# asmirnou/watsor

Measured on NVIDIA H100. Metric: aggregate detection FPS on synthetic 640x480 streams, higher is better.
Workload: dtype f32

## Files before the change

### watsor_b200/csrc/kernels_tc.cu

```cuda
#include <cuda.h>

#include <algorithm>
#include <cstdlib>
#include <cstring>

#include "kernels_tc.cuh"
#include "tc_common.cuh"

namespace {

struct TcArgs {
  const float* scale;
  const float* offset;
  void* out;
  float* enc;
  float* logits;
  int M, N, n_pad, K;
  int block_n, stages, k_blocks;
  int splits, kb_per;
  float* partial;
  int* tile_counters;
  const void* residual;
  int conv, cpb, conv_kw, conv_pad_t, conv_pad_l;
  int ring_bytes;
  int rows_per_tile;
  int act, is_head, anchors_per_loc, row_off, n_box, num_anchors, ncp1, hw;
};

__device__ __forceinline__ void tma_load_4d_tc(uint32_t dst, const CUtensorMap* map, uint32_t bar, int c0, int c1, int c2,
                                               int c3) {
  asm volatile(
      "cp.async.bulk.tensor.4d.shared::cluster.global.mbarrier::complete_tx::bytes [%0], [%1, {%3, %4, %5, %6}], [%2];" ::
          "r"(dst),
      "l"(map), "r"(bar), "r"(c0), "r"(c1), "r"(c2), "r"(c3)
      : "memory");
}

__device__ __forceinline__ void cluster_sync_all() {
  asm volatile("barrier.cluster.arrive.release.aligned;\nbarrier.cluster.wait.acquire.aligned;" ::: "memory");
}
__device__ __forceinline__ uint32_t cluster_ctarank() {
  uint32_t r;
  asm volatile("mov.u32 %0, %%cluster_ctarank;" : "=r"(r));
  return r;
}
__device__ __forceinline__ float4 ld_dsmem128(uint32_t addr, uint32_t rank) {
  uint32_t ra;
  asm volatile("mapa.shared::cluster.u32 %0, %1, %2;" : "=r"(ra) : "r"(addr), "r"(rank));
  float4 v;
  asm volatile("ld.shared::cluster.v4.f32 {%0,%1,%2,%3}, [%4];" : "=f"(v.x), "=f"(v.y), "=f"(v.z), "=f"(v.w) : "r"(ra));
  return v;
}

template <bool TF32>
__device__ __forceinline__ void copy_out_row(const TcArgs& g, const uint8_t* smem, int pitch, int r, int m0, int n0,
                                             int lane, int members, int reduce) {
  const int mm = m0 + r;
  const uint32_t src = smem_u32(smem) + (uint32_t)(r * pitch * 4);
  size_t hr = 0;
  if (g.is_head) {
    const int f = mm / g.hw;
    hr = (size_t)f * g.num_anchors + g.row_off + (size_t)(mm - f * g.hw) * g.anchors_per_loc;
  }
  for (int j = lane * 4; j < g.block_n; j += 128) {
    const int nn = n0 + j;
    if (nn >= g.N) break;
    float4 y;
    if (reduce) {
      float4 p[8];
      if (members == 1) {
        p[0] = lds128(src + (uint32_t)(j * 4));
      } else {
#pragma unroll
        for (int z = 0; z < 8; ++z)
          if (z < members) p[z] = ld_dsmem128(src + (uint32_t)(j * 4), (uint32_t)z);
      }
      y = p[0];
#pragma unroll
      for (int z = 1; z < 8; ++z)
        if (z < members) y = make_float4(__fadd_rn(y.x, p[z].x), __fadd_rn(y.y, p[z].y), __fadd_rn(y.z, p[z].z), __fadd_rn(y.w, p[z].w));
      const float4 sc = *reinterpret_cast<const float4*>(g.scale + nn), of = *reinterpret_cast<const float4*>(g.offset + nn);
      y = make_float4(affine_rn(y.x, sc.x, of.x), affine_rn(y.y, sc.y, of.y), affine_rn(y.z, sc.z, of.z), affine_rn(y.w, sc.w, of.w));
      if (g.act == WB_ACT_RELU6) y = make_float4(relu6f(y.x), relu6f(y.y), relu6f(y.z), relu6f(y.w));
    } else {
      y = lds128(src + (uint32_t)(j * 4));
    }
    if (g.is_head) {
      const float ys[4] = {y.x, y.y, y.z, y.w};
#pragma unroll
      for (int e = 0; e < 4; ++e) {
        const int c = nn + e;
        if (c >= g.N) break;
        if (c < g.n_box)
          g.enc[hr * 4 + c] = ys[e];
        else
          g.logits[hr * g.ncp1 + (c - g.n_box)] = ys[e];
      }
    } else if (TF32) {
      if (g.residual != nullptr) {
        const float4 rr = *reinterpret_cast<const float4*>(reinterpret_cast<const float*>(g.residual) + (size_t)mm * g.N + nn);
        y = make_float4(__fadd_rn(y.x, rr.x), __fadd_rn(y.y, rr.y), __fadd_rn(y.z, rr.z), __fadd_rn(y.w, rr.w));
      }
      *reinterpret_cast<float4*>(reinterpret_cast<float*>(g.out) + (size_t)mm * g.N + nn) = y;
    } else {
      ActIO<__nv_bfloat16>::st4(reinterpret_cast<__nv_bfloat16*>(g.out) + (size_t)mm * g.N + nn, y);
    }
  }
}

constexpr int GEMM_THREADS = 288;
constexpr int GEMM_PRODUCER_WARP = 8;

__device__ __forceinline__ void wg_bar_sync(int wg) { asm volatile("bar.sync %0, 128;" ::"r"(2 + wg) : "memory"); }

template <int MODE, int BN>
__global__ void __launch_bounds__(GEMM_THREADS, 1)
    k_gemm_tc(const __grid_constant__ CUtensorMap map_a, const __grid_constant__ CUtensorMap map_b,
              const __grid_constant__ CUtensorMap map_b_lo, TcArgs g) {
  constexpr bool TF32 = MODE != 0;
  constexpr bool X3 = MODE == 2;
  constexpr int ELEM = TF32 ? 4 : 2;
  constexpr int K_PER_BLOCK = ROW_BYTES / ELEM;
  constexpr int B_TILE_BYTES = BN * ROW_BYTES;
  constexpr int SLOTS = X3 ? 2 : 1;
  constexpr int STAGE_BYTES = (A_TILE_BYTES + B_TILE_BYTES) * SLOTS;
  extern __shared__ __align__(1024) uint8_t smem_raw[];
  uint8_t* smem = reinterpret_cast<uint8_t*>((reinterpret_cast<uintptr_t>(smem_raw) + 1023) & ~(uintptr_t)1023);
  uint64_t* full = reinterpret_cast<uint64_t*>(smem + (size_t)g.ring_bytes);
  uint64_t* empty = full + g.stages;

  const int warp = threadIdx.x >> 5, lane = threadIdx.x & 31;
  const int m0 = blockIdx.x * g.rows_per_tile, n0 = blockIdx.y * BN;
  const int kb0 = blockIdx.z * g.kb_per;
  const int nkb = min(g.k_blocks, kb0 + g.kb_per) - kb0;

  if (threadIdx.x == 0) {
    for (int s = 0; s < g.stages; ++s) {
      mbar_init(smem_u32(&full[s]), 1);
      mbar_init(smem_u32(&empty[s]), 2);
    }
    fence_barrier_init();
  }
  __syncthreads();

  float acc[BN / 2];
#pragma unroll
  for (int i = 0; i < BN / 2; ++i) acc[i] = 0.f;

  if (warp == GEMM_PRODUCER_WARP) {
    if (elect_one()) {
      asm volatile("prefetch.tensormap [%0];" ::"l"(&map_a) : "memory");
      asm volatile("prefetch.tensormap [%0];" ::"l"(&map_b) : "memory");
      for (int it = 0; it < nkb; ++it) {
        const int kb = kb0 + it;
        const int s = it % g.stages;
        const uint32_t ph = (it / g.stages) & 1;
        mbar_wait(smem_u32(&empty[s]), ph ^ 1);
        uint8_t* st = smem + (size_t)s * STAGE_BYTES;
        const uint32_t bar = smem_u32(&full[s]);
        if (g.conv) {
          mbar_expect_tx(bar, g.rows_per_tile * ROW_BYTES + B_TILE_BYTES * SLOTS);
          const int tap = kb / g.cpb, cb = kb - tap * g.cpb;
          const int ky = tap / g.conv_kw, kx = tap - ky * g.conv_kw;
          tma_load_4d_tc(smem_u32(st), &map_a, bar, cb * K_PER_BLOCK, kx - g.conv_pad_l, ky - g.conv_pad_t, m0 / g.hw);
        } else {
          mbar_expect_tx(bar, A_TILE_BYTES + B_TILE_BYTES * SLOTS);
          tma_load_2d(smem_u32(st), &map_a, bar, kb * K_PER_BLOCK, m0);
        }
        uint8_t* sb = st + A_TILE_BYTES * SLOTS;
        tma_load_2d(smem_u32(sb), &map_b, bar, kb * K_PER_BLOCK, n0);
        if (X3) tma_load_2d(smem_u32(sb + B_TILE_BYTES), &map_b_lo, bar, kb * K_PER_BLOCK, n0);
      }
    }
  } else {
    const int wg = warp >> 2, t = threadIdx.x & 127;
    float part[X3 ? BN / 2 : 1];
    for (int it = 0; it < nkb; ++it) {
      const int s = it % g.stages;
      mbar_wait(smem_u32(&full[s]), (it / g.stages) & 1);
      const uint32_t st = smem_u32(smem + (size_t)s * STAGE_BYTES);
      const uint32_t a_hi = st + (uint32_t)(wg * 64 * ROW_BYTES), a_lo = a_hi + A_TILE_BYTES;
      const uint32_t b_hi = st + (uint32_t)(A_TILE_BYTES * SLOTS), b_lo = b_hi + B_TILE_BYTES;
      if (X3) {
#pragma unroll
        for (int i = t; i < 64 * ROW_BYTES / 16; i += 128) split_tf32(a_hi + (uint32_t)(i * 16), a_lo + (uint32_t)(i * 16));
        fence_proxy_async();
        wg_bar_sync(wg);
        wg_x3_kblock_sum<BN>(acc, part, a_hi, a_lo, b_hi, b_lo);
      } else {
        wgmma_fence();
        wg_mma_kblock<TF32, false, BN>(acc, a_hi, a_lo, b_hi, b_lo, 1u);
        wgmma_commit();
        wgmma_wait_all();
      }
      wg_bar_sync(wg);
      if (t == 0) mbar_arrive(smem_u32(&empty[s]));
    }
  }

  const int pitch = BN + 4;
  __syncthreads();
  if (warp < GEMM_PRODUCER_WARP) {
    const int row = (warp >> 2) * 64 + (warp & 3) * 16 + (lane >> 2);
    const uint32_t stg = smem_u32(smem) + (uint32_t)((row * pitch + 2 * (lane & 3)) * 4);
#pragma unroll
    for (int i = 0; i < BN / 2; i += 4) {
      const uint32_t c = (uint32_t)((i >> 2) * 8 * 4);
      asm volatile("st.shared.v2.f32 [%0], {%1, %2};" ::"r"(stg + c), "f"(acc[i]), "f"(acc[i + 1]) : "memory");
      asm volatile("st.shared.v2.f32 [%0], {%1, %2};" ::"r"(stg + c + (uint32_t)(8 * pitch * 4)), "f"(acc[i + 2]), "f"(acc[i + 3])
                   : "memory");
    }
  }
  __syncthreads();
  const int n_warps = blockDim.x >> 5;
  const int rows = min(g.rows_per_tile, g.M - m0);
  if (g.splits > 1) {
    cluster_sync_all();
    const int z = (int)cluster_ctarank();
    for (int r = z + g.splits * warp; r < rows; r += n_warps * g.splits)
      copy_out_row<TF32>(g, smem, pitch, r, m0, n0, lane, g.splits, 1);
    __syncwarp();
    cluster_sync_all();
  } else if (g.is_head) {
    for (int r = warp; r < rows; r += n_warps) copy_out_row<TF32>(g, smem, pitch, r, m0, n0, lane, 1, 1);
  } else {
    const int c4n = g.block_n >> 2;
    const int items = rows * c4n;
    const int T = (int)blockDim.x;
    const uint32_t sbase = smem_u32(smem);
    int inc_r = T / c4n, inc_c = T - inc_r * c4n;
    int r_it = (int)threadIdx.x / c4n, c_it = (int)threadIdx.x - r_it * c4n;
    if (TF32 && inc_r >= 1) {
      inc_c = 0;
      if ((int)threadIdx.x >= inc_r * c4n) r_it = rows;
    }
    if (inc_c == 0 && TF32) {
      const int nn = n0 + c_it * 4;
      if (nn < g.N && r_it < rows) {
        const float4 sc = __ldg(reinterpret_cast<const float4*>(g.scale + nn)), of = __ldg(reinterpret_cast<const float4*>(g.offset + nn));
        const bool relu = g.act == WB_ACT_RELU6;
        uint32_t sp = sbase + (uint32_t)((r_it * pitch + c_it * 4) * 4);
        const uint32_t sstep = (uint32_t)(inc_r * pitch * 4);
        float* op = reinterpret_cast<float*>(g.out) + (size_t)(m0 + r_it) * g.N + nn;
        const float* rp = g.residual != nullptr ? reinterpret_cast<const float*>(g.residual) + (size_t)(m0 + r_it) * g.N + nn : nullptr;
        const size_t gstep = (size_t)inc_r * g.N;
        int r = r_it;
        for (; r + 3 * inc_r < rows; r += 4 * inc_r) {
          float4 y[4], rs[4];
#pragma unroll
          for (int u = 0; u < 4; ++u) {
            y[u] = lds128(sp + u * sstep);
            if (rp != nullptr) rs[u] = *reinterpret_cast<const float4*>(rp + u * gstep);
          }
#pragma unroll
          for (int u = 0; u < 4; ++u) {
            float4 v = make_float4(affine_rn(y[u].x, sc.x, of.x), affine_rn(y[u].y, sc.y, of.y), affine_rn(y[u].z, sc.z, of.z),
                                   affine_rn(y[u].w, sc.w, of.w));
            if (relu) v = make_float4(relu6f(v.x), relu6f(v.y), relu6f(v.z), relu6f(v.w));
            if (rp != nullptr) v = make_float4(__fadd_rn(v.x, rs[u].x), __fadd_rn(v.y, rs[u].y), __fadd_rn(v.z, rs[u].z), __fadd_rn(v.w, rs[u].w));
            *reinterpret_cast<float4*>(op + u * gstep) = v;
          }
          sp += 4 * sstep;
          op += 4 * gstep;
          if (rp != nullptr) rp += 4 * gstep;
        }
        for (; r < rows; r += inc_r) {
          const float4 y = lds128(sp);
          float4 v = make_float4(affine_rn(y.x, sc.x, of.x), affine_rn(y.y, sc.y, of.y), affine_rn(y.z, sc.z, of.z), affine_rn(y.w, sc.w, of.w));
          if (relu) v = make_float4(relu6f(v.x), relu6f(v.y), relu6f(v.z), relu6f(v.w));
          if (rp != nullptr) {
            const float4 r4 = *reinterpret_cast<const float4*>(rp);
            v = make_float4(__fadd_rn(v.x, r4.x), __fadd_rn(v.y, r4.y), __fadd_rn(v.z, r4.z), __fadd_rn(v.w, r4.w));
            rp += gstep;
          }
          *reinterpret_cast<float4*>(op) = v;
          sp += sstep;
          op += gstep;
        }
      }
    } else
    for (int i0 = threadIdx.x; i0 < items; i0 += 4 * T) {
      float4 y[4], sc[4], of[4];
      int rr[4], cc[4];
#pragma unroll
      for (int u = 0; u < 4; ++u) {
        rr[u] = r_it;
        cc[u] = c_it * 4;
        if (i0 + T * u < items && n0 + cc[u] < g.N) {
          y[u] = lds128(sbase + (uint32_t)((rr[u] * pitch + cc[u]) * 4));
          sc[u] = __ldg(reinterpret_cast<const float4*>(g.scale + n0 + cc[u]));
          of[u] = __ldg(reinterpret_cast<const float4*>(g.offset + n0 + cc[u]));
        }
        r_it += inc_r;
        c_it += inc_c;
        if (c_it >= c4n) {
          c_it -= c4n;
          ++r_it;
        }
      }
#pragma unroll
      for (int u = 0; u < 4; ++u) {
        const int nn = n0 + cc[u];
        if (i0 + T * u >= items || nn >= g.N) continue;
        const size_t o = (size_t)(m0 + rr[u]) * g.N + nn;
        y[u] = make_float4(affine_rn(y[u].x, sc[u].x, of[u].x), affine_rn(y[u].y, sc[u].y, of[u].y),
                           affine_rn(y[u].z, sc[u].z, of[u].z), affine_rn(y[u].w, sc[u].w, of[u].w));
        if (g.act == WB_ACT_RELU6) y[u] = make_float4(relu6f(y[u].x), relu6f(y[u].y), relu6f(y[u].z), relu6f(y[u].w));
        if (TF32) {
          if (g.residual != nullptr) {
            const float4 r4 = *reinterpret_cast<const float4*>(reinterpret_cast<const float*>(g.residual) + o);
            y[u] = make_float4(__fadd_rn(y[u].x, r4.x), __fadd_rn(y[u].y, r4.y), __fadd_rn(y[u].z, r4.z), __fadd_rn(y[u].w, r4.w));
          }
          *reinterpret_cast<float4*>(reinterpret_cast<float*>(g.out) + o) = y[u];
        } else {
          ActIO<__nv_bfloat16>::st4(reinterpret_cast<__nv_bfloat16*>(g.out) + o, y[u]);
        }
      }
    }
  }
}


typedef CUresult (*EncodeTiledFn)(CUtensorMap*, CUtensorMapDataType, cuuint32_t, void*, const cuuint64_t*,
                                  const cuuint64_t*, const cuuint32_t*, const cuuint32_t*, CUtensorMapInterleave,
                                  CUtensorMapSwizzle, CUtensorMapL2promotion, CUtensorMapFloatOOBfill);

EncodeTiledFn encode_fn() {
  static EncodeTiledFn fn = nullptr;
  if (!fn) {
    void* p = nullptr;
    cudaDriverEntryPointQueryResult q;
    if (cudaGetDriverEntryPoint("cuTensorMapEncodeTiled", &p, cudaEnableDefault, &q) == cudaSuccess &&
        q == cudaDriverEntryPointSuccess)
      fn = reinterpret_cast<EncodeTiledFn>(p);
  }
  return fn;
}

bool make_map(CUtensorMap* map, const void* base, int elem_bytes, int rows, int k, int box_rows, std::string* err) {
  EncodeTiledFn fn = encode_fn();
  if (!fn) {
    *err = "cuTensorMapEncodeTiled is not available from the driver";
    return false;
  }
  cuuint64_t dims[2] = {(cuuint64_t)k, (cuuint64_t)rows};
  cuuint64_t strides[1] = {(cuuint64_t)k * elem_bytes};
  cuuint32_t box[2] = {(cuuint32_t)(ROW_BYTES / elem_bytes), (cuuint32_t)box_rows};
  cuuint32_t estr[2] = {1, 1};
  CUresult r = fn(map, elem_bytes == 2 ? CU_TENSOR_MAP_DATA_TYPE_BFLOAT16 : CU_TENSOR_MAP_DATA_TYPE_FLOAT32, 2,
                  const_cast<void*>(base), dims, strides, box, estr, CU_TENSOR_MAP_INTERLEAVE_NONE,
                  CU_TENSOR_MAP_SWIZZLE_128B, CU_TENSOR_MAP_L2_PROMOTION_L2_256B, CU_TENSOR_MAP_FLOAT_OOB_FILL_NONE);
  if (r != CUDA_SUCCESS) {
    *err = "cuTensorMapEncodeTiled failed with code " + std::to_string((int)r) + " (rows " + std::to_string(rows) +
           ", k " + std::to_string(k) + ", box_rows " + std::to_string(box_rows) + ")";
    return false;
  }
  return true;
}

}

bool tc_encode_map(void* map, const void* base, int elem_bytes, int rank, const unsigned long long* dims,
                   const unsigned long long* strides_bytes, const unsigned* box, bool swizzle128, std::string* err,
                   const unsigned* elem_strides) {
  EncodeTiledFn fn = encode_fn();
  if (!fn) {
    *err = "cuTensorMapEncodeTiled is not available from the driver";
    return false;
  }
  cuuint64_t d[5], st[4];
  cuuint32_t b[5], es[5];
  for (int i = 0; i < rank; ++i) {
    d[i] = dims[i];
    b[i] = box[i];
    es[i] = elem_strides ? elem_strides[i] : 1;
    if (i + 1 < rank) st[i] = strides_bytes[i];
  }
  CUresult r = fn(reinterpret_cast<CUtensorMap*>(map),
                  elem_bytes == 2 ? CU_TENSOR_MAP_DATA_TYPE_BFLOAT16 : CU_TENSOR_MAP_DATA_TYPE_FLOAT32, (cuuint32_t)rank,
                  const_cast<void*>(base), d, st, b, es, CU_TENSOR_MAP_INTERLEAVE_NONE,
                  swizzle128 ? CU_TENSOR_MAP_SWIZZLE_128B : CU_TENSOR_MAP_SWIZZLE_NONE, CU_TENSOR_MAP_L2_PROMOTION_L2_256B,
                  CU_TENSOR_MAP_FLOAT_OOB_FILL_NONE);
  if (r != CUDA_SUCCESS) {
    *err = "cuTensorMapEncodeTiled (rank " + std::to_string(rank) + ") failed with code " + std::to_string((int)r);
    return false;
  }
  return true;
}

namespace {

int num_sms_hint() {
  static int n = 0;
  if (n == 0) {
    int dev = 0;
    cudaGetDevice(&dev);
    cudaDeviceGetAttribute(&n, cudaDevAttrMultiProcessorCount, dev);
    if (n <= 0) n = 132;
  }
  return n;
}

int pick_block_n(int n_pad) { return n_pad <= 32 ? 32 : (n_pad <= 64 ? 64 : 128); }

}

bool tc_layer_supported(const wb_layer& L) {
  if ((L.op == WB_OP_PW || L.op == WB_OP_HEAD) && L.kh == 1 && L.kw == 1 && L.stride == 1 && L.in_c % 4 == 0) return true;
  return L.op == WB_OP_CONV && L.in_c % 64 == 0 && L.out_h * L.out_w <= (uint32_t)BLOCK_M && L.stride <= 8 &&
         getenv("WB_NO_TC_CONV") == nullptr;
}

int tc_prepare_weights(const std::vector<wb_layer>& layers, const std::vector<wb_tensor_entry>& tensors,
                       const float* host_data, int mode, TcWeights* out, std::string* err) {
  out->mode = mode;
  out->layers.assign(layers.size(), TcLayerWeights{});
  for (size_t li = 0; li < layers.size(); ++li) {
    const wb_layer& L = layers[li];
    if (!tc_layer_supported(L)) continue;
    TcLayerWeights& w = out->layers[li];
    const int K = L.kh * L.kw * L.in_c, NP = L.n_pad;
    const float* src = host_data + tensors[L.w_tensor].offset;
    w.k = K;
    w.n_pad = NP;
    w.block_n = pick_block_n(NP);
    const int elem = mode == TC_BF16 ? 2 : 4;
    const size_t bytes = (size_t)NP * K * elem;
    std::vector<uint8_t> hi(bytes), lo(mode == TC_TF32X3 ? bytes : 0);
    for (int n = 0; n < NP; ++n)
      for (int k = 0; k < K; ++k) {
        float v = src[(size_t)k * NP + n];
        if (mode == TC_BF16) {
          __nv_bfloat16 b = __float2bfloat16_rn(v);
          memcpy(&hi[((size_t)n * K + k) * 2], &b, 2);
        } else {
          uint32_t u;
          memcpy(&u, &v, 4);
          uint32_t h = mode == TC_TF32X3 ? (u & 0xFFFFE000u) : u;
          memcpy(&hi[((size_t)n * K + k) * 4], &h, 4);
          if (mode == TC_TF32X3) {
            float hf;
            memcpy(&hf, &h, 4);
            float lf = v - hf;
            uint32_t l;
            memcpy(&l, &lf, 4);
            l &= 0xFFFFE000u;
            memcpy(&lo[((size_t)n * K + k) * 4], &l, 4);
          }
        }
      }
    if (cudaMalloc(&w.w, bytes) != cudaSuccess || cudaMemcpy(w.w, hi.data(), bytes, cudaMemcpyHostToDevice) != cudaSuccess) {
      *err = "cudaMalloc/cudaMemcpy of tensor-core weights failed";
      return 1;
    }
    if (!make_map(reinterpret_cast<CUtensorMap*>(w.tmap_b), w.w, elem, NP, K, w.block_n, err)) return 1;
    if (mode == TC_TF32X3) {
      if (cudaMalloc(&w.w_lo, bytes) != cudaSuccess ||
          cudaMemcpy(w.w_lo, lo.data(), bytes, cudaMemcpyHostToDevice) != cudaSuccess) {
        *err = "cudaMalloc/cudaMemcpy of tensor-core weights failed";
        return 1;
      }
      if (!make_map(reinterpret_cast<CUtensorMap*>(w.tmap_b_lo), w.w_lo, elem, NP, K, w.block_n, err)) return 1;
    } else {
      memcpy(w.tmap_b_lo, w.tmap_b, sizeof(w.tmap_b));
    }
    w.ready = true;
  }
  return 0;
}

void tc_free_weights(TcWeights* w) {
  for (auto& l : w->layers) {
    if (l.w) cudaFree(l.w);
    if (l.w_lo) cudaFree(l.w_lo);
  }
  w->layers.clear();
}

int tc_launch_gemm(const LaunchCtx& lc, const TcWeights& tw, int layer_index, int n, const wb_layer& L, const void* in,
                   const float* scale, const float* offset, void* out, float* enc, float* logits, int num_anchors,
                   int num_classes_p1, float* partial, size_t partial_floats, int* tile_counters, const void* residual,
                   std::string* err) {
  const TcLayerWeights& w = tw.layers[layer_index];
  if (!w.ready) {
    *err = "no tensor-core weights for this layer";
    return 1;
  }
  const int mode = tw.mode;
  const int elem = mode == TC_BF16 ? 2 : 4;
  TcArgs g;
  g.scale = scale;
  g.offset = offset;
  g.out = out;
  g.enc = enc;
  g.logits = logits;
  g.M = n * L.out_h * L.out_w;
  g.N = L.out_c;
  g.n_pad = L.n_pad;
  g.K = L.kh * L.kw * L.in_c;
  g.block_n = w.block_n;
  g.tile_counters = tile_counters;
  g.residual = mode == TC_BF16 ? nullptr : residual;
  g.conv = L.op == WB_OP_CONV;
  g.cpb = (L.in_c * elem) / ROW_BYTES;
  g.conv_kw = L.kw;
  g.conv_pad_t = L.pad_t;
  g.conv_pad_l = L.pad_l;
  g.rows_per_tile = g.conv ? (BLOCK_M / (int)(L.out_h * L.out_w)) * (int)(L.out_h * L.out_w) : BLOCK_M;
  if (mode == TC_BF16 && residual != nullptr) {
    *err = "residual fusion is not available in bf16 mode";
    return 1;
  }
  g.k_blocks = (g.K * elem + ROW_BYTES - 1) / ROW_BYTES;
  g.act = L.act;
  g.is_head = L.op == WB_OP_HEAD;
  g.anchors_per_loc = L.anchors_per_loc;
  g.row_off = L.row_off;
  g.n_box = L.n_box;
  g.num_anchors = num_anchors;
  g.ncp1 = num_classes_p1;
  g.hw = L.out_h * L.out_w;
  const int x3 = mode == TC_TF32X3 ? 2 : 1;
  const int stage_bytes = (A_TILE_BYTES + g.block_n * ROW_BYTES) * x3;
  dim3 grid((g.M + g.rows_per_tile - 1) / g.rows_per_tile, (g.n_pad + g.block_n - 1) / g.block_n);
  g.splits = 1;
  g.kb_per = g.k_blocks;
  g.partial = partial;
  const long tiles = (long)grid.x * grid.y;
  if (tiles < num_sms_hint() / 2 && g.k_blocks >= 16 && getenv("WB_NO_SPLITK") == nullptr) {
    int want = std::max(1, (int)(num_sms_hint() / tiles));
    int splits = std::min(std::min(want, g.k_blocks / 8), 8);
    if (splits > 1) {
      g.kb_per = (g.k_blocks + splits - 1) / splits;
      g.splits = (g.k_blocks + g.kb_per - 1) / g.kb_per;
      grid.z = g.splits;
    }
  }
  int stages = std::min(6, (200 * 1024) / stage_bytes);
  if (stages > g.kb_per) stages = g.kb_per;
  if (stages < 1) stages = 1;
  g.stages = stages;
  const int staging = BLOCK_M * (g.block_n + 4) * 4;
  g.ring_bytes = ((std::max(stages * stage_bytes, staging) + 1023) / 1024) * 1024;
  const size_t smem = (size_t)g.ring_bytes + 1024  + 16 * stages;
  alignas(64) CUtensorMap map_a;
  if (g.conv) {
    const int imgs = BLOCK_M / (int)(L.out_h * L.out_w);
    unsigned long long dims[4] = {L.in_c, L.in_w, L.in_h, (unsigned long long)n};
    unsigned long long st[3] = {(unsigned long long)L.in_c * elem, (unsigned long long)L.in_w * L.in_c * elem,
                                (unsigned long long)L.in_h * L.in_w * L.in_c * elem};
    unsigned box[4] = {(unsigned)(ROW_BYTES / elem), (unsigned)((L.out_w - 1) * L.stride + 1),
                       (unsigned)((L.out_h - 1) * L.stride + 1), (unsigned)imgs};
    unsigned es[4] = {1, L.stride, L.stride, 1};
    if (!tc_encode_map(&map_a, in, elem, 4, dims, st, box, true, err, es)) return 1;
  } else if (!make_map(&map_a, in, elem, g.M, g.K, BLOCK_M, err)) {
    return 1;
  }
  CUtensorMap map_b, map_b_lo;
  memcpy(&map_b, w.tmap_b, sizeof(map_b));
  memcpy(&map_b_lo, w.tmap_b_lo, sizeof(map_b_lo));
  auto launch = [&](auto kern, PerDeviceFlag& attr_done) {
    if (!attr_done.get()) {
      cudaError_t e = cudaFuncSetAttribute(kern, cudaFuncAttributeMaxDynamicSharedMemorySize, 227 * 1024);
      if (e != cudaSuccess) return e;
      attr_done.set();
    }
    cudaLaunchConfig_t cfg = {};
    cfg.gridDim = grid;
    cfg.blockDim = dim3(GEMM_THREADS);
    cfg.dynamicSmemBytes = smem;
    cfg.stream = lc.stream;
    cudaLaunchAttribute at[1];
    at[0].id = cudaLaunchAttributeClusterDimension;
    at[0].val.clusterDim.x = 1;
    at[0].val.clusterDim.y = 1;
    at[0].val.clusterDim.z = (unsigned)g.splits;
    cfg.attrs = at;
    cfg.numAttrs = g.splits > 1 ? 1 : 0;
    return cudaLaunchKernelEx(&cfg, kern, map_a, map_b, map_b_lo, g);
  };
  static PerDeviceFlag attr_done[3][3];
  const int bi = g.block_n == 32 ? 0 : (g.block_n == 64 ? 1 : 2);
  cudaError_t e;
  if (mode == TC_BF16) {
    e = bi == 0 ? launch(k_gemm_tc<0, 32>, attr_done[0][0])
                : (bi == 1 ? launch(k_gemm_tc<0, 64>, attr_done[0][1]) : launch(k_gemm_tc<0, 128>, attr_done[0][2]));
  } else if (mode == TC_TF32X1) {
    e = bi == 0 ? launch(k_gemm_tc<1, 32>, attr_done[1][0])
                : (bi == 1 ? launch(k_gemm_tc<1, 64>, attr_done[1][1]) : launch(k_gemm_tc<1, 128>, attr_done[1][2]));
  } else {
    e = bi == 0 ? launch(k_gemm_tc<2, 32>, attr_done[2][0])
                : (bi == 1 ? launch(k_gemm_tc<2, 64>, attr_done[2][1]) : launch(k_gemm_tc<2, 128>, attr_done[2][2]));
  }
  if (e != cudaSuccess) {
    *err = std::string("tensor-core GEMM launch: ") + cudaGetErrorString(e);
    return 1;
  }
  ++*lc.launch_counter;
  return 0;
}
```

Before: 12220.

## Add persistent tile-looping GEMM kernel with separate epilogue staging buffer

When there are more output tiles than SMs and no split-K, the GEMM now launches a persistent grid sized by occupancy. Each CTA loops over tiles, keeping the TMA producer running ahead into the next tile while consumers run the epilogue in a dedicated staging area synchronised only among consumer warps. For BN=32 it also targets two CTAs per SM by shrinking the smem budget, and the non-persistent epilogue is refactored into a shared function with compile-time column counts. The aim is to cut launch/tail overhead and overlap epilogue stores with next-tile loads, at the cost of fewer pipeline stages and extra register pressure.

```diff
diff --git a/watsor_b200/csrc/kernels_tc.cu b/watsor_b200/csrc/kernels_tc.cu
--- a/watsor_b200/csrc/kernels_tc.cu
+++ b/watsor_b200/csrc/kernels_tc.cu
@@ -3,6 +3,7 @@
 #include <algorithm>
 #include <cstdlib>
 #include <cstring>
+#include <type_traits>
 
 #include "kernels_tc.cuh"
 #include "tc_common.cuh"
@@ -22,8 +23,10 @@
   int* tile_counters;
   const void* residual;
   int conv, cpb, conv_kw, conv_pad_t, conv_pad_l;
-  int ring_bytes;
+  int staging_off;
+  int bar_off;
   int rows_per_tile;
+  int tiles, tiles_n;
   int act, is_head, anchors_per_loc, row_off, n_box, num_anchors, ncp1, hw;
 };
 
@@ -110,11 +113,94 @@
 
 constexpr int GEMM_THREADS = 288;
 constexpr int GEMM_PRODUCER_WARP = 8;
+constexpr int GEMM_CONSUMER_THREADS = 32 * GEMM_PRODUCER_WARP;
 
 __device__ __forceinline__ void wg_bar_sync(int wg) { asm volatile("bar.sync %0, 128;" ::"r"(2 + wg) : "memory"); }
-
-template <int MODE, int BN>
-__global__ void __launch_bounds__(GEMM_THREADS, 1)
+template <int THREADS>
+__device__ __forceinline__ void epilogue_bar_sync() {
+  if (THREADS == GEMM_THREADS)
+    __syncthreads();
+  else
+    asm volatile("bar.sync 1, %0;" ::"n"(THREADS) : "memory");
+}
+
+template <bool TF32, int BN, int THREADS>
+__device__ __forceinline__ void gemm_epilogue(const TcArgs& g, const float* acc, uint8_t* stg, int m0, int n0, int warp,
+                                              int lane) {
+  const int pitch = BN + 4;
+  epilogue_bar_sync<THREADS>();
+  if (warp < GEMM_PRODUCER_WARP) {
+    const int row = (warp >> 2) * 64 + (warp & 3) * 16 + (lane >> 2);
+    const uint32_t s = smem_u32(stg) + (uint32_t)((row * pitch + 2 * (lane & 3)) * 4);
+#pragma unroll
+    for (int i = 0; i < BN / 2; i += 4) {
+      const uint32_t c = (uint32_t)((i >> 2) * 8 * 4);
+      asm volatile("st.shared.v2.f32 [%0], {%1, %2};" ::"r"(s + c), "f"(acc[i]), "f"(acc[i + 1]) : "memory");
+      asm volatile("st.shared.v2.f32 [%0], {%1, %2};" ::"r"(s + c + (uint32_t)(8 * pitch * 4)), "f"(acc[i + 2]), "f"(acc[i + 3])
+                   : "memory");
+    }
+  }
+  epilogue_bar_sync<THREADS>();
+  constexpr int n_warps = THREADS >> 5;
+  const int rows = min(g.rows_per_tile, g.M - m0);
+  if (g.splits > 1) {
+    cluster_sync_all();
+    const int z = (int)cluster_ctarank();
+    for (int r = z + g.splits * warp; r < rows; r += n_warps * g.splits)
+      copy_out_row<TF32>(g, stg, pitch, r, m0, n0, lane, g.splits, 1);
+    __syncwarp();
+    cluster_sync_all();
+  } else if (g.is_head) {
+    for (int r = warp; r < rows; r += n_warps) copy_out_row<TF32>(g, stg, pitch, r, m0, n0, lane, 1, 1);
+  } else {
+    constexpr int C4N = BN / 4;
+    constexpr int INC_R = THREADS / C4N;
+    static_assert(THREADS % C4N == 0, "a row of float4 columns divides the epilogue's threads");
+    const int r_it = (int)threadIdx.x / C4N, c_it = (int)threadIdx.x % C4N;
+    const int nn = n0 + c_it * 4;
+    if (nn < g.N && r_it < rows) {
+      const float4 sc = __ldg(reinterpret_cast<const float4*>(g.scale + nn)), of = __ldg(reinterpret_cast<const float4*>(g.offset + nn));
+      const bool relu = g.act == WB_ACT_RELU6;
+      uint32_t sp = smem_u32(stg) + (uint32_t)((r_it * pitch + c_it * 4) * 4);
+      constexpr uint32_t sstep = (uint32_t)(INC_R * pitch * 4);
+      size_t o = (size_t)(m0 + r_it) * g.N + nn;
+      const size_t gstep = (size_t)INC_R * g.N;
+      const float* res = TF32 ? reinterpret_cast<const float*>(g.residual) : nullptr;
+      auto finish = [&](float4 y, size_t at, float4 r4) {
+        float4 v = make_float4(affine_rn(y.x, sc.x, of.x), affine_rn(y.y, sc.y, of.y), affine_rn(y.z, sc.z, of.z), affine_rn(y.w, sc.w, of.w));
+        if (relu) v = make_float4(relu6f(v.x), relu6f(v.y), relu6f(v.z), relu6f(v.w));
+        if (res != nullptr) v = make_float4(__fadd_rn(v.x, r4.x), __fadd_rn(v.y, r4.y), __fadd_rn(v.z, r4.z), __fadd_rn(v.w, r4.w));
+        if (TF32)
+          *reinterpret_cast<float4*>(reinterpret_cast<float*>(g.out) + at) = v;
+        else
+          ActIO<__nv_bfloat16>::st4(reinterpret_cast<__nv_bfloat16*>(g.out) + at, v);
+      };
+      int r = r_it;
+      for (; r + 3 * INC_R < rows; r += 4 * INC_R) {
+        float4 y[4], rs[4] = {};
+#pragma unroll
+        for (int u = 0; u < 4; ++u) {
+          y[u] = lds128(sp + u * sstep);
+          if (res != nullptr) rs[u] = *reinterpret_cast<const float4*>(res + o + u * gstep);
+        }
+#pragma unroll
+        for (int u = 0; u < 4; ++u) finish(y[u], o + u * gstep, rs[u]);
+        sp += 4 * sstep;
+        o += 4 * gstep;
+      }
+      for (; r < rows; r += INC_R) {
+        float4 r4 = make_float4(0.f, 0.f, 0.f, 0.f);
+        if (res != nullptr) r4 = *reinterpret_cast<const float4*>(res + o);
+        finish(lds128(sp), o, r4);
+        sp += sstep;
+        o += gstep;
+      }
+    }
+  }
+}
+
+template <int MODE, int BN, bool PERSIST>
+__global__ void __launch_bounds__(GEMM_THREADS, PERSIST && BN == 32 ? 2 : 1)
     k_gemm_tc(const __grid_constant__ CUtensorMap map_a, const __grid_constant__ CUtensorMap map_b,
               const __grid_constant__ CUtensorMap map_b_lo, TcArgs g) {
   constexpr bool TF32 = MODE != 0;
@@ -126,11 +212,10 @@
   constexpr int STAGE_BYTES = (A_TILE_BYTES + B_TILE_BYTES) * SLOTS;
   extern __shared__ __align__(1024) uint8_t smem_raw[];
   uint8_t* smem = reinterpret_cast<uint8_t*>((reinterpret_cast<uintptr_t>(smem_raw) + 1023) & ~(uintptr_t)1023);
-  uint64_t* full = reinterpret_cast<uint64_t*>(smem + (size_t)g.ring_bytes);
+  uint64_t* full = reinterpret_cast<uint64_t*>(smem + (size_t)g.bar_off);
   uint64_t* empty = full + g.stages;
 
   const int warp = threadIdx.x >> 5, lane = threadIdx.x & 31;
-  const int m0 = blockIdx.x * g.rows_per_tile, n0 = blockIdx.y * BN;
   const int kb0 = blockIdx.z * g.kb_per;
   const int nkb = min(g.k_blocks, kb0 + g.kb_per) - kb0;
 
@@ -151,172 +236,74 @@
     if (elect_one()) {
       asm volatile("prefetch.tensormap [%0];" ::"l"(&map_a) : "memory");
       asm volatile("prefetch.tensormap [%0];" ::"l"(&map_b) : "memory");
-      for (int it = 0; it < nkb; ++it) {
-        const int kb = kb0 + it;
-        const int s = it % g.stages;
-        const uint32_t ph = (it / g.stages) & 1;
-        mbar_wait(smem_u32(&empty[s]), ph ^ 1);
-        uint8_t* st = smem + (size_t)s * STAGE_BYTES;
-        const uint32_t bar = smem_u32(&full[s]);
-        if (g.conv) {
-          mbar_expect_tx(bar, g.rows_per_tile * ROW_BYTES + B_TILE_BYTES * SLOTS);
-          const int tap = kb / g.cpb, cb = kb - tap * g.cpb;
-          const int ky = tap / g.conv_kw, kx = tap - ky * g.conv_kw;
-          tma_load_4d_tc(smem_u32(st), &map_a, bar, cb * K_PER_BLOCK, kx - g.conv_pad_l, ky - g.conv_pad_t, m0 / g.hw);
-        } else {
-          mbar_expect_tx(bar, A_TILE_BYTES + B_TILE_BYTES * SLOTS);
-          tma_load_2d(smem_u32(st), &map_a, bar, kb * K_PER_BLOCK, m0);
+      int it = 0;
+      for (int tile = blockIdx.x; tile < g.tiles; tile += gridDim.x) {
+        const int mt = tile / g.tiles_n;
+        const int m0 = mt * g.rows_per_tile, n0 = (tile - mt * g.tiles_n) * BN;
+        for (int i = 0; i < nkb; ++i, ++it) {
+          const int kb = kb0 + i;
+          const int s = it % g.stages;
+          const uint32_t ph = (it / g.stages) & 1;
+          mbar_wait(smem_u32(&empty[s]), ph ^ 1);
+          uint8_t* st = smem + (size_t)s * STAGE_BYTES;
+          const uint32_t bar = smem_u32(&full[s]);
+          if (g.conv) {
+            mbar_expect_tx(bar, g.rows_per_tile * ROW_BYTES + B_TILE_BYTES * SLOTS);
+            const int tap = kb / g.cpb, cb = kb - tap * g.cpb;
+            const int ky = tap / g.conv_kw, kx = tap - ky * g.conv_kw;
+            tma_load_4d_tc(smem_u32(st), &map_a, bar, cb * K_PER_BLOCK, kx - g.conv_pad_l, ky - g.conv_pad_t, m0 / g.hw);
+          } else {
+            mbar_expect_tx(bar, A_TILE_BYTES + B_TILE_BYTES * SLOTS);
+            tma_load_2d(smem_u32(st), &map_a, bar, kb * K_PER_BLOCK, m0);
+          }
+          uint8_t* sb = st + A_TILE_BYTES * SLOTS;
+          tma_load_2d(smem_u32(sb), &map_b, bar, kb * K_PER_BLOCK, n0);
+          if (X3) tma_load_2d(smem_u32(sb + B_TILE_BYTES), &map_b_lo, bar, kb * K_PER_BLOCK, n0);
         }
-        uint8_t* sb = st + A_TILE_BYTES * SLOTS;
-        tma_load_2d(smem_u32(sb), &map_b, bar, kb * K_PER_BLOCK, n0);
-        if (X3) tma_load_2d(smem_u32(sb + B_TILE_BYTES), &map_b_lo, bar, kb * K_PER_BLOCK, n0);
-      }
-    }
+        if (!PERSIST) break;
+      }
+    }
+    __syncwarp();
   } else {
     const int wg = warp >> 2, t = threadIdx.x & 127;
-    float part[X3 ? BN / 2 : 1];
-    for (int it = 0; it < nkb; ++it) {
-      const int s = it % g.stages;
-      mbar_wait(smem_u32(&full[s]), (it / g.stages) & 1);
-      const uint32_t st = smem_u32(smem + (size_t)s * STAGE_BYTES);
-      const uint32_t a_hi = st + (uint32_t)(wg * 64 * ROW_BYTES), a_lo = a_hi + A_TILE_BYTES;
-      const uint32_t b_hi = st + (uint32_t)(A_TILE_BYTES * SLOTS), b_lo = b_hi + B_TILE_BYTES;
-      if (X3) {
-#pragma unroll
-        for (int i = t; i < 64 * ROW_BYTES / 16; i += 128) split_tf32(a_hi + (uint32_t)(i * 16), a_lo + (uint32_t)(i * 16));
-        fence_proxy_async();
+    int it = 0;
+    for (int tile = blockIdx.x; tile < g.tiles; tile += gridDim.x) {
+      const int mt = tile / g.tiles_n;
+      const int m0 = mt * g.rows_per_tile, n0 = (tile - mt * g.tiles_n) * BN;
+      float part[X3 ? BN / 2 : 1];
+      if (PERSIST) {
+#pragma unroll
+        for (int i = 0; i < BN / 2; ++i) acc[i] = 0.f;
+      }
+      for (int i = 0; i < nkb; ++i, ++it) {
+        const int s = it % g.stages;
+        mbar_wait(smem_u32(&full[s]), (it / g.stages) & 1);
+        const uint32_t st = smem_u32(smem + (size_t)s * STAGE_BYTES);
+        const uint32_t a_hi = st + (uint32_t)(wg * 64 * ROW_BYTES), a_lo = a_hi + A_TILE_BYTES;
+        const uint32_t b_hi = st + (uint32_t)(A_TILE_BYTES * SLOTS), b_lo = b_hi + B_TILE_BYTES;
+        if (X3) {
+#pragma unroll
+          for (int c = t; c < 64 * ROW_BYTES / 16; c += 128) split_tf32(a_hi + (uint32_t)(c * 16), a_lo + (uint32_t)(c * 16));
+          fence_proxy_async();
+          wg_bar_sync(wg);
+          wg_x3_kblock_sum<BN>(acc, part, a_hi, a_lo, b_hi, b_lo);
+        } else {
+          wgmma_fence();
+          wg_mma_kblock<TF32, false, BN>(acc, a_hi, a_lo, b_hi, b_lo, 1u);
+          wgmma_commit();
+          wgmma_wait_all();
+        }
         wg_bar_sync(wg);
-        wg_x3_kblock_sum<BN>(acc, part, a_hi, a_lo, b_hi, b_lo);
-      } else {
-        wgmma_fence();
-        wg_mma_kblock<TF32, false, BN>(acc, a_hi, a_lo, b_hi, b_lo, 1u);
-        wgmma_commit();
-        wgmma_wait_all();
-      }
-      wg_bar_sync(wg);
-      if (t == 0) mbar_arrive(smem_u32(&empty[s]));
-    }
-  }
-
-  const int pitch = BN + 4;
-  __syncthreads();
-  if (warp < GEMM_PRODUCER_WARP) {
-    const int row = (warp >> 2) * 64 + (warp & 3) * 16 + (lane >> 2);
-    const uint32_t stg = smem_u32(smem) + (uint32_t)((row * pitch + 2 * (lane & 3)) * 4);
-#pragma unroll
-    for (int i = 0; i < BN / 2; i += 4) {
-      const uint32_t c = (uint32_t)((i >> 2) * 8 * 4);
-      asm volatile("st.shared.v2.f32 [%0], {%1, %2};" ::"r"(stg + c), "f"(acc[i]), "f"(acc[i + 1]) : "memory");
-      asm volatile("st.shared.v2.f32 [%0], {%1, %2};" ::"r"(stg + c + (uint32_t)(8 * pitch * 4)), "f"(acc[i + 2]), "f"(acc[i + 3])
-                   : "memory");
-    }
-  }
-  __syncthreads();
-  const int n_warps = blockDim.x >> 5;
-  const int rows = min(g.rows_per_tile, g.M - m0);
-  if (g.splits > 1) {
-    cluster_sync_all();
-    const int z = (int)cluster_ctarank();
-    for (int r = z + g.splits * warp; r < rows; r += n_warps * g.splits)
-      copy_out_row<TF32>(g, smem, pitch, r, m0, n0, lane, g.splits, 1);
-    __syncwarp();
-    cluster_sync_all();
-  } else if (g.is_head) {
-    for (int r = warp; r < rows; r += n_warps) copy_out_row<TF32>(g, smem, pitch, r, m0, n0, lane, 1, 1);
-  } else {
-    const int c4n = g.block_n >> 2;
-    const int items = rows * c4n;
-    const int T = (int)blockDim.x;
-    const uint32_t sbase = smem_u32(smem);
-    int inc_r = T / c4n, inc_c = T - inc_r * c4n;
-    int r_it = (int)threadIdx.x / c4n, c_it = (int)threadIdx.x - r_it * c4n;
-    if (TF32 && inc_r >= 1) {
-      inc_c = 0;
-      if ((int)threadIdx.x >= inc_r * c4n) r_it = rows;
-    }
-    if (inc_c == 0 && TF32) {
-      const int nn = n0 + c_it * 4;
-      if (nn < g.N && r_it < rows) {
-        const float4 sc = __ldg(reinterpret_cast<const float4*>(g.scale + nn)), of = __ldg(reinterpret_cast<const float4*>(g.offset + nn));
-        const bool relu = g.act == WB_ACT_RELU6;
-        uint32_t sp = sbase + (uint32_t)((r_it * pitch + c_it * 4) * 4);
-        const uint32_t sstep = (uint32_t)(inc_r * pitch * 4);
-        float* op = reinterpret_cast<float*>(g.out) + (size_t)(m0 + r_it) * g.N + nn;
-        const float* rp = g.residual != nullptr ? reinterpret_cast<const float*>(g.residual) + (size_t)(m0 + r_it) * g.N + nn : nullptr;
-        const size_t gstep = (size_t)inc_r * g.N;
-        int r = r_it;
-        for (; r + 3 * inc_r < rows; r += 4 * inc_r) {
-          float4 y[4], rs[4];
-#pragma unroll
-          for (int u = 0; u < 4; ++u) {
-            y[u] = lds128(sp + u * sstep);
-            if (rp != nullptr) rs[u] = *reinterpret_cast<const float4*>(rp + u * gstep);
-          }
-#pragma unroll
-          for (int u = 0; u < 4; ++u) {
-            float4 v = make_float4(affine_rn(y[u].x, sc.x, of.x), affine_rn(y[u].y, sc.y, of.y), affine_rn(y[u].z, sc.z, of.z),
-                                   affine_rn(y[u].w, sc.w, of.w));
-            if (relu) v = make_float4(relu6f(v.x), relu6f(v.y), relu6f(v.z), relu6f(v.w));
-            if (rp != nullptr) v = make_float4(__fadd_rn(v.x, rs[u].x), __fadd_rn(v.y, rs[u].y), __fadd_rn(v.z, rs[u].z), __fadd_rn(v.w, rs[u].w));
-            *reinterpret_cast<float4*>(op + u * gstep) = v;
-          }
-          sp += 4 * sstep;
-          op += 4 * gstep;
-          if (rp != nullptr) rp += 4 * gstep;
-        }
-        for (; r < rows; r += inc_r) {
-          const float4 y = lds128(sp);
-          float4 v = make_float4(affine_rn(y.x, sc.x, of.x), affine_rn(y.y, sc.y, of.y), affine_rn(y.z, sc.z, of.z), affine_rn(y.w, sc.w, of.w));
-          if (relu) v = make_float4(relu6f(v.x), relu6f(v.y), relu6f(v.z), relu6f(v.w));
-          if (rp != nullptr) {
-            const float4 r4 = *reinterpret_cast<const float4*>(rp);
-            v = make_float4(__fadd_rn(v.x, r4.x), __fadd_rn(v.y, r4.y), __fadd_rn(v.z, r4.z), __fadd_rn(v.w, r4.w));
-            rp += gstep;
-          }
-          *reinterpret_cast<float4*>(op) = v;
-          sp += sstep;
-          op += gstep;
-        }
-      }
-    } else
-    for (int i0 = threadIdx.x; i0 < items; i0 += 4 * T) {
-      float4 y[4], sc[4], of[4];
-      int rr[4], cc[4];
-#pragma unroll
-      for (int u = 0; u < 4; ++u) {
-        rr[u] = r_it;
-        cc[u] = c_it * 4;
-        if (i0 + T * u < items && n0 + cc[u] < g.N) {
-          y[u] = lds128(sbase + (uint32_t)((rr[u] * pitch + cc[u]) * 4));
-          sc[u] = __ldg(reinterpret_cast<const float4*>(g.scale + n0 + cc[u]));
-          of[u] = __ldg(reinterpret_cast<const float4*>(g.offset + n0 + cc[u]));
-        }
-        r_it += inc_r;
-        c_it += inc_c;
-        if (c_it >= c4n) {
-          c_it -= c4n;
-          ++r_it;
-        }
-      }
-#pragma unroll
-      for (int u = 0; u < 4; ++u) {
-        const int nn = n0 + cc[u];
-        if (i0 + T * u >= items || nn >= g.N) continue;
-        const size_t o = (size_t)(m0 + rr[u]) * g.N + nn;
-        y[u] = make_float4(affine_rn(y[u].x, sc[u].x, of[u].x), affine_rn(y[u].y, sc[u].y, of[u].y),
-                           affine_rn(y[u].z, sc[u].z, of[u].z), affine_rn(y[u].w, sc[u].w, of[u].w));
-        if (g.act == WB_ACT_RELU6) y[u] = make_float4(relu6f(y[u].x), relu6f(y[u].y), relu6f(y[u].z), relu6f(y[u].w));
-        if (TF32) {
-          if (g.residual != nullptr) {
-            const float4 r4 = *reinterpret_cast<const float4*>(reinterpret_cast<const float*>(g.residual) + o);
-            y[u] = make_float4(__fadd_rn(y[u].x, r4.x), __fadd_rn(y[u].y, r4.y), __fadd_rn(y[u].z, r4.z), __fadd_rn(y[u].w, r4.w));
-          }
-          *reinterpret_cast<float4*>(reinterpret_cast<float*>(g.out) + o) = y[u];
-        } else {
-          ActIO<__nv_bfloat16>::st4(reinterpret_cast<__nv_bfloat16*>(g.out) + o, y[u]);
-        }
-      }
-    }
+        if (t == 0) mbar_arrive(smem_u32(&empty[s]));
+      }
+      if (!PERSIST) break;
+      gemm_epilogue<TF32, BN, GEMM_CONSUMER_THREADS>(g, acc, smem + g.staging_off, m0, n0, warp, lane);
+    }
+  }
+  if (!PERSIST) {
+    const int mt = blockIdx.x / g.tiles_n;
+    gemm_epilogue<TF32, BN, GEMM_THREADS>(g, acc, smem, mt * g.rows_per_tile, (blockIdx.x - mt * g.tiles_n) * BN, warp,
+                                          lane);
   }
 }
 
@@ -522,11 +509,13 @@
   g.hw = L.out_h * L.out_w;
   const int x3 = mode == TC_TF32X3 ? 2 : 1;
   const int stage_bytes = (A_TILE_BYTES + g.block_n * ROW_BYTES) * x3;
-  dim3 grid((g.M + g.rows_per_tile - 1) / g.rows_per_tile, (g.n_pad + g.block_n - 1) / g.block_n);
+  g.tiles_n = (g.n_pad + g.block_n - 1) / g.block_n;
+  g.tiles = ((g.M + g.rows_per_tile - 1) / g.rows_per_tile) * g.tiles_n;
+  dim3 grid(g.tiles);
   g.splits = 1;
   g.kb_per = g.k_blocks;
   g.partial = partial;
-  const long tiles = (long)grid.x * grid.y;
+  const long tiles = g.tiles;
   if (tiles < num_sms_hint() / 2 && g.k_blocks >= 16 && getenv("WB_NO_SPLITK") == nullptr) {
     int want = std::max(1, (int)(num_sms_hint() / tiles));
     int splits = std::min(std::min(want, g.k_blocks / 8), 8);
@@ -536,13 +525,22 @@
       grid.z = g.splits;
     }
   }
-  int stages = std::min(6, (200 * 1024) / stage_bytes);
-  if (stages > g.kb_per) stages = g.kb_per;
-  if (stages < 1) stages = 1;
+  const int staging = BLOCK_M * (g.block_n + 4) * 4;
+  const bool persistent = g.splits == 1 && tiles > num_sms_hint();
+  int stages;
+  if (!persistent) {
+    stages = std::max(1, std::min(std::min(6, (200 * 1024) / stage_bytes), g.kb_per));
+    g.staging_off = 0;
+    g.bar_off = ((std::max(stages * stage_bytes, staging) + 1023) / 1024) * 1024;
+  } else {
+    const int half = 110 * 1024;
+    const int budget = 2 * stage_bytes + staging <= half ? half : 200 * 1024;
+    stages = std::max(2, std::min(6, (budget - staging) / stage_bytes));
+    g.staging_off = stages * stage_bytes;
+    g.bar_off = g.staging_off + staging;
+  }
   g.stages = stages;
-  const int staging = BLOCK_M * (g.block_n + 4) * 4;
-  g.ring_bytes = ((std::max(stages * stage_bytes, staging) + 1023) / 1024) * 1024;
-  const size_t smem = (size_t)g.ring_bytes + 1024  + 16 * stages;
+  const size_t smem = (size_t)g.bar_off + 1024  + 16 * stages;
   alignas(64) CUtensorMap map_a;
   if (g.conv) {
     const int imgs = BLOCK_M / (int)(L.out_h * L.out_w);
@@ -564,6 +562,12 @@
       cudaError_t e = cudaFuncSetAttribute(kern, cudaFuncAttributeMaxDynamicSharedMemorySize, 227 * 1024);
       if (e != cudaSuccess) return e;
       attr_done.set();
+    }
+    if (persistent) {
+      int per_sm = 0;
+      cudaError_t e = cudaOccupancyMaxActiveBlocksPerMultiprocessor(&per_sm, kern, GEMM_THREADS, smem);
+      if (e != cudaSuccess) return e;
+      grid.x = (unsigned)std::min<long>(tiles, (long)num_sms_hint() * std::max(1, per_sm));
     }
     cudaLaunchConfig_t cfg = {};
     cfg.gridDim = grid;
@@ -579,19 +583,18 @@
     cfg.numAttrs = g.splits > 1 ? 1 : 0;
     return cudaLaunchKernelEx(&cfg, kern, map_a, map_b, map_b_lo, g);
   };
-  static PerDeviceFlag attr_done[3][3];
+  static PerDeviceFlag attr_done[3][3][2];
   const int bi = g.block_n == 32 ? 0 : (g.block_n == 64 ? 1 : 2);
-  cudaError_t e;
-  if (mode == TC_BF16) {
-    e = bi == 0 ? launch(k_gemm_tc<0, 32>, attr_done[0][0])
-                : (bi == 1 ? launch(k_gemm_tc<0, 64>, attr_done[0][1]) : launch(k_gemm_tc<0, 128>, attr_done[0][2]));
-  } else if (mode == TC_TF32X1) {
-    e = bi == 0 ? launch(k_gemm_tc<1, 32>, attr_done[1][0])
-                : (bi == 1 ? launch(k_gemm_tc<1, 64>, attr_done[1][1]) : launch(k_gemm_tc<1, 128>, attr_done[1][2]));
-  } else {
-    e = bi == 0 ? launch(k_gemm_tc<2, 32>, attr_done[2][0])
-                : (bi == 1 ? launch(k_gemm_tc<2, 64>, attr_done[2][1]) : launch(k_gemm_tc<2, 128>, attr_done[2][2]));
-  }
+  auto launch_mode = [&](auto mode_c) {
+    constexpr int M = decltype(mode_c)::value;
+    PerDeviceFlag* f = attr_done[M][bi];
+    if (bi == 0) return persistent ? launch(k_gemm_tc<M, 32, true>, f[1]) : launch(k_gemm_tc<M, 32, false>, f[0]);
+    if (bi == 1) return persistent ? launch(k_gemm_tc<M, 64, true>, f[1]) : launch(k_gemm_tc<M, 64, false>, f[0]);
+    return persistent ? launch(k_gemm_tc<M, 128, true>, f[1]) : launch(k_gemm_tc<M, 128, false>, f[0]);
+  };
+  const cudaError_t e = mode == TC_BF16     ? launch_mode(std::integral_constant<int, 0>())
+                        : mode == TC_TF32X1 ? launch_mode(std::integral_constant<int, 1>())
+                                            : launch_mode(std::integral_constant<int, 2>());
   if (e != cudaSuccess) {
     *err = std::string("tensor-core GEMM launch: ") + cudaGetErrorString(e);
     return 1;
```

Result: faster. 12840 (median of 6 runs) (+5.1%).
